# rebots-online/InstantIR

Measured on AMD Instinct MI355X. Metric: denoising steps/sec at 1024x1024 (InstantIR step: previewer UNet + LCM + Aggregator + UNet, CFG), higher is better.
Workload: dtype f16 (fp32 accumulate)

## Files before the change

### instantir_amd/csrc/gemm_conv.hip

```cpp
#include "common.h"
#include "gemm_geo.h"
#include "../../include/instantir_hip.h"
#include <stdlib.h>
#include <type_traits>

namespace {

using iir::Geo;

constexpr int BK = 64;
#ifndef IIR_NO_PIN
#define IIR_PIN() __builtin_amdgcn_sched_barrier(0)
#else
#define IIR_PIN() ((void)0)
#endif
constexpr int PF_TOUCHES = 4;
#define IIR_DEFAULT_STAGES 2
#ifndef IIR_T1_MIN
#define IIR_T1_MIN 384
#endif
#ifndef IIR_T2_MIN
#define IIR_T2_MIN 256
#endif


__device__ __forceinline__ void ln_merge(float& n, float& mean, float& m2, float nb, float mb, float m2b) {
    const float tot = n + nb, d = mb - mean;
    mean += d * (nb / tot);
    m2 += m2b + d * d * (n * nb / tot);
    n = tot;
}

constexpr int vmcnt_imm(int n) { return (n & 15) | 0x0F70 | ((n >> 4) << 14); }

template <int N>
__device__ __forceinline__ void wait_vm_lgkm_and_barrier() {
#ifdef IIR_DBG_NO_BARRIER
    asm volatile("s_waitcnt vmcnt(%0) lgkmcnt(0)" ::"n"(N) : "memory");
#else
    asm volatile("s_waitcnt vmcnt(%0) lgkmcnt(0)\n\ts_barrier" ::"n"(N) : "memory");
#endif
}

template <int N>
__device__ __forceinline__ void wait_vm_and_barrier() {
#ifdef IIR_DBG_NO_BARRIER
    asm volatile("s_waitcnt vmcnt(%0)" ::"n"(N) : "memory");
#else
    asm volatile("s_waitcnt vmcnt(%0)\n\ts_barrier" ::"n"(N) : "memory");
#endif
}

template <typename E, int BM, int BN, int ST, bool CONV, int WAVES_M = 2, bool W8 = false, bool LW = false, bool F8 = false>
__global__ __launch_bounds__(128 * WAVES_M * (LW ? 2 : 1), (WAVES_M == 2 ? 2 : 1)) void gemm_kernel(const Geo g) {
    static_assert(!(F8 && (W8 || CONV)), "the all-fp8 build covers the linear layers; W8 is the fp16-activation form");
    static_assert(!(W8 && CONV), "the fp8-weight build covers the linear layers only");
    static_assert(!(LW && W8), "loader waves: fp16 / bf16 operands only");
    using E4 = typename ET<E>::x4;
    using E8 = typename ET<E>::x8;
    constexpr int NW = WAVES_M * 2;
    constexpr int NT = 64 * NW * (LW ? 2 : 1);
    constexpr int WM = BM / WAVES_M, WN = BN / 2;
    constexpr int MI = WM / 16, NI = WN / 16;
    constexpr int B_GROUPS = W8 ? BN / 16 : BN / 8;
    constexpr int A_INST = BM / 8 / NW, B_INST = (B_GROUPS + NW - 1) / NW;
    constexpr int B_STAGE_BYTES = W8 ? BN * 64 : BN * 128;
    constexpr int RING_BYTES = ST * (BM * 128 + B_STAGE_BYTES);
    extern __shared__ __attribute__((aligned(16))) char smem[];
    f16* As = (f16*)smem;
    f16* Bs = As + ST * BM * BK;
    constexpr int LOADS = A_INST + B_INST;
    constexpr int SCRATCH_BYTES = 256 * NW * (LW ? 2 : 1);
    float2* rowstat = (float2*)(smem + RING_BYTES + SCRATCH_BYTES);
    constexpr int LNP_OFF = (BM * (2 * BN + 32) + 15) / 16 * 16;
    constexpr bool LN_OUT_FITS = LNP_OFF + BM * (BN / 8) * 8 <= RING_BYTES;
    constexpr int GN_RG = NT / (BN / 8);
    constexpr bool GN_OUT_FITS = BM % 64 == 0 && LNP_OFF + GN_RG * BN * 8 <= RING_BYTES && BN <= NT;

    const int tid = threadIdx.x;
    const int lane = tid & 63;
    const int wave_all = __builtin_amdgcn_readfirstlane(tid >> 6);
    const bool loader = LW && wave_all >= NW;
    const int wave = loader ? wave_all - NW : wave_all;
    const int wm = wave >> 1, wn = wave & 1;

    const int kz = (g.splitk == 2 && blockIdx.x >= (gridDim.x >> 1)) ? 1 : 0;
    int tm, tn;
    {
        const int bid = kz ? (int)blockIdx.x - (int)(gridDim.x >> 1) : (int)blockIdx.x, xcd = bid & 7, local = bid >> 3;
        const int rx = xcd % g.xm, ry = xcd / g.xm;
        tm = rx * g.rm + local % g.rm;
        tn = ry * g.rn + local / g.rm;
        if (tm >= g.tiles_m || tn >= g.tiles_n) return;
    }
    const int m0 = tm * BM, n0 = tn * BN;

    const int srow = lane >> 3;
    const int schunk = (lane & 7) ^ srow;
    const f16* a_src[A_INST];
    int a_pix_y[A_INST], a_pix_x[A_INST];
    const f16* a_img[A_INST];
#pragma unroll
    for (int i = 0; i < A_INST; ++i) {
        int m = m0 + (i * NW + wave) * 8 + srow;
        if (m >= g.M) m = g.M - 1;
        if (!CONV) {
            a_src[i] = g.A + (long)m * g.lda + schunk * 8;
        } else {
            const int hw = g.Ho * g.Wo;
            const int img = m / hw, rem = m - img * hw;
            const int oy = rem / g.Wo, ox = rem - oy * g.Wo;
            a_img[i] = g.A + (long)img * g.x_img_stride + schunk * 8;
            a_pix_y[i] = oy * g.stride - g.pad;
            a_pix_x[i] = ox * g.stride - g.pad;
        }
    }
    const f16* b_src[B_INST];
#pragma unroll
    for (int i = 0; i < B_INST; ++i) {
        if (!W8) {
            int n = n0 + (i * NW + wave) * 8 + srow;
            if (n >= g.N) n = g.N - 1;
            b_src[i] = g.W + (long)n * g.K + schunk * 8;
        } else {
            const int r = (i * NW + wave) * 16 + (lane >> 2);
            int n = n0 + r;
            if (n >= g.N) n = g.N - 1;
            b_src[i] = (const f16*)((const char*)g.W + (long)n * g.K + (((lane & 3) ^ ((r >> 2) & 3)) * 16));
        }
    }

    const f16* cv_ptr[CONV ? A_INST : 1];
    int cv_inc[CONV ? A_INST : 1];
    int cv_c0 = 0, cv_tap = 0;
    auto conv_tap = [&](int tap) {
        const int ky = tap / g.ks, kx = tap - ky * g.ks;
#pragma unroll
        for (int i = 0; i < (CONV ? A_INST : 0); ++i) {
            const int iy = a_pix_y[i] + ky, ix = a_pix_x[i] + kx;
            bool ok;
            long pix;
            if (g.ups) {
                ok = (iy >= 0) & (iy < 2 * g.H) & (ix >= 0) & (ix < 2 * g.Wd);
                pix = (long)(iy >> 1) * g.Wd + (ix >> 1);
            } else {
                ok = (iy >= 0) & (iy < g.H) & (ix >= 0) & (ix < g.Wd);
                pix = (long)iy * g.Wd + ix;
            }
            cv_ptr[i] = ok ? a_img[i] + pix * g.lda : g.zero + (lane & 7) * 8;
            cv_inc[i] = ok ? BK : 0;
        }
    };
    auto conv_seek = [&](int kt) {
        const int k0 = kt * BK;
        cv_tap = k0 / g.Cin;
        cv_c0 = k0 - cv_tap * g.Cin;
        conv_tap(cv_tap);
#pragma unroll
        for (int i = 0; i < (CONV ? A_INST : 0); ++i) cv_ptr[i] += cv_inc[i] ? cv_c0 : 0;
    };
// ... 466 lines not shown
    } else {
#pragma unroll
        for (int j = 0; j < NI; ++j) {
            const int n = n0 + wn * WN + j * 16 + fq * 4;
            const bool in_n = n < g.N;
            float sc[4] = {1.f, 1.f, 1.f, 1.f}, c0[4] = {0.f, 0.f, 0.f, 0.f}, c1[4] = {0.f, 0.f, 0.f, 0.f};
            if ((W8 || F8) && in_n) { const f32x4 ws = *(const f32x4*)(g.wscale + n); for (int t = 0; t < 4; ++t) sc[t] = ws[t] * g.a_scale; }
            for (int t = 0; t < 4; ++t) { c1[t] = pre_c1[j][t]; c0[t] = (float)pre_c0[j][t]; }
#pragma unroll
            for (int i = 0; i < MI; ++i) {
                const int lr = lrs[i];
                float a[4];
                for (int t = 0; t < 4; ++t) a[t] = (W8 || F8) ? acc[i][j][t] * sc[t] : acc[i][j][t];
                for (int t = 0; t < 4; ++t) a[t] = fmaf(a[t], rss[i].x, fmaf(rss[i].y, c1[t], c0[t]));
                float b[4];
                for (int t = 0; t < 4; ++t) b[t] = __shfl_xor(a[t], 32, 64);
                if (g.epi == IIR_EPI_GEGLU) {
                    if (!in_n) continue;
                    const bool gate = fq >= 2;
                    const int lco = (wn * WN + j * 16) / 2 + (fq & 1) * 4 + (gate ? 2 : 0);
                    const float v0 = gate ? b[2] : a[0], v1 = gate ? b[3] : a[1], g0 = gate ? a[2] : b[0], g1 = gate ? a[3] : b[1];
                    typedef E E2 __attribute__((ext_vector_type(2)));
                    E2 o2 = {(E)(v0 * gelu_erf_f(g0)), (E)(v1 * gelu_erf_f(g1))};
                    *(E2*)(ct + lr * cs + lco * 2) = o2;
                    continue;
                }
                if (fq >= 2 || !in_n) continue;
                const int lco = (wn * WN + j * 16) / 2 + fq * 4;
                long mr = ms[i];
                if (CONV && g.res_img_rows) { const int hw = g.Ho * g.Wo, img = ms[i] / hw; mr = (long)img * g.res_img_rows + (ms[i] - img * hw); }
                E4 o;
                {
                    E4 h = *(const E4*)(g.res + mr * g.ldr + n0 / 2 + lco);
                    for (int t = 0; t < 4; ++t) o[t] = (E)((float)h[t] * (a[t] + 1.0f) + b[t]);
                }
                *(E4*)(ct + lr * cs + lco * 2) = o;
            }
        }
    }
    }
    asm volatile("s_waitcnt lgkmcnt(0)\n\ts_barrier" ::: "memory");

    auto touch_next_weights = [&]() {
#ifdef IIR_DBG_NO_TOUCH
        return;
#endif
        const int per = (g.pf_lines + (int)gridDim.x - 1) / (int)gridDim.x;
        const long l0 = (long)blockIdx.x * per, last = g.pf_lines - 1;
        char* scratch = smem + RING_BYTES + wave_all * 256;
#pragma unroll
        for (int i = 0; i < PF_TOUCHES; ++i) {
            long l = l0 + min(tid + i * NT, per - 1);
            if (l > last) l = last;
            __builtin_amdgcn_global_load_lds((const GLOBAL_AS void*)(g.pf + l * 128), (LDS_AS void*)scratch, 4, 0, 0);
        }
    };
    auto write_out = [&](auto cpr_tag) {
        constexpr int CPR = decltype(cpr_tag)::value;
        constexpr int TOTAL = BM * CPR, CH = (TOTAL + NT - 1) / NT;
        const int no_tile = paired ? n0 / 2 : n0, No = paired ? g.N / 2 : g.N;
        const bool use_res = g.res && !paired;
        const bool remap = CONV && (g.y_img_rows | g.res_img_rows);
        const bool tr_tile = g.Ct && no_tile >= g.tr_from;
        const bool tr_mixed = g.Ct && !tr_tile && no_tile + CPR * 8 > g.tr_from;
        const bool inside = m0 + BM <= g.M && no_tile + CPR * 8 <= No && !remap;
        const bool fast = !tr_tile && !tr_mixed && g.c_vec && (!use_res || g.r_vec) && inside;
        if (tr_tile && inside && g.ct_vec && !use_res) {
            constexpr int RC = BM / 8, TOTAL_T = (CPR * 8) * RC, CH_T = (TOTAL_T + NT - 1) / NT;
            touch_next_weights();
#pragma unroll
            for (int k = 0; k < CH_T; ++k) {
                const int idx = tid + k * NT;
                if (TOTAL_T % NT != 0 && idx >= TOTAL_T) break;
                const int c = idx / RC, rc = idx - c * RC;
                E8 o;
#pragma unroll
                for (int t = 0; t < 8; ++t) o[t] = (E)((float)*(const E*)(ct + (rc * 8 + t) * cs + c * 2) * g.out_scale);
                *(E8*)(g.Ct + (long)(no_tile + c - g.tr_from) * g.ldct + m0 + rc * 8) = o;
            }
            return;
        }
        if constexpr (GN_OUT_FITS && CPR == BN / 8) {
        if (fast && g.gn_out && !paired) {
            constexpr int RG = NT / CPR, RPT = (64 + RG - 1) / RG;
            const int cc = tid % CPR, rg = tid / CPR;
            const bool active = rg < RG;
            float2* part = (float2*)(smem + LNP_OFF);
            touch_next_weights();
#pragma unroll 1
            for (int half = 0; half < BM / 64; ++half) {
                E8 rr[RPT];
                if (use_res) {
#pragma unroll
                    for (int j = 0; j < RPT; ++j) {
                        const int r = half * 64 + min(rg + j * RG, 63);
                        rr[j] = *(const E8*)(g.res + (long)(m0 + r) * g.ldr + no_tile + min(cc, CPR - 1) * 8);
                    }
                }
                float k0[8], s8[8], q8[8];
#pragma unroll
                for (int t = 0; t < 8; ++t) { k0[t] = 0.f; s8[t] = 0.f; q8[t] = 0.f; }
                int cnt = 0;
#pragma unroll
                for (int j = 0; j < RPT; ++j) {
                    const int rl = rg + j * RG;
                    if (active && rl < 64) {
                        const int r = half * 64 + rl;
                        const E8 v = *(const E8*)(ct + r * cs + cc * 16);
                        E8 o;
                        for (int t = 0; t < 8; ++t) o[t] = (E)(((float)v[t] + (use_res ? (float)rr[j][t] : 0.f)) * g.out_scale);
                        iir::store16(g.C, ((long)(m0 + r) * g.ldc + no_tile + cc * 8) * 2, o, g.st_wt != 0);
                        for (int t = 0; t < 8; ++t) {
                            const float f = (float)o[t];
                            if (j == 0) k0[t] = f;
                            const float d = f - k0[t];
                            s8[t] += d; q8[t] = fmaf(d, d, q8[t]);
                        }
                        ++cnt;
                    }
                }
                if (active) {
                    const float inv = 1.0f / (float)cnt;
#pragma unroll
                    for (int t = 0; t < 8; ++t)
                        part[rg * BN + cc * 8 + t] = make_float2(k0[t] + s8[t] * inv, fmaxf(q8[t] - s8[t] * s8[t] * inv, 0.f));
                }
                __syncthreads();
                if (tid < BN) {
                    float n = 0.f, mean = 0.f, m2 = 0.f;
#pragma unroll 4
                    for (int q = 0; q < RG; ++q) {
                        const float2 pq = part[q * BN + tid];
                        const float nb = (float)((64 - q + RG - 1) / RG);
                        const float tot = n + nb, d = pq.x - mean;
                        mean += d * (nb / tot);
                        m2 += pq.y + d * d * (n * nb / tot);
                        n = tot;
                    }
                    ((float2*)g.gn_out)[(long)(m0 / 64 + half) * g.N + n0 + tid] = make_float2(mean, m2);
                }
                __syncthreads();
            }
            return;
        }
        }
        if (fast) {
            E8 o[CH];
            if (use_res) {
                E8 rr[CH];
#pragma unroll
                for (int k = 0; k < CH; ++k) {
                    const int c = min(tid + k * NT, TOTAL - 1), r = c / CPR, cc = c - r * CPR;
                    rr[k] = *(const E8*)(g.res + (long)(m0 + r) * g.ldr + no_tile + cc * 8);
                }
#pragma unroll
                for (int k = 0; k < CH; ++k) {
                    const int c = min(tid + k * NT, TOTAL - 1), r = c / CPR, cc = c - r * CPR;
                    const E8 v = *(const E8*)(ct + r * cs + cc * 16);
                    for (int t = 0; t < 8; ++t) o[k][t] = (E)(((float)v[t] + (float)rr[k][t]) * g.out_scale);
                }
            } else {
#pragma unroll
                for (int k = 0; k < CH; ++k) {
                    const int c = min(tid + k * NT, TOTAL - 1), r = c / CPR, cc = c - r * CPR;
                    const E8 v = *(const E8*)(ct + r * cs + cc * 16);
                    for (int t = 0; t < 8; ++t) o[k][t] = (E)((float)v[t] * g.out_scale);
                }
            }
            touch_next_weights();
#pragma unroll
            for (int k = 0; k < CH; ++k) {
                const int c = tid + k * NT, r = c / CPR, cc = c - r * CPR;
                if (TOTAL % NT != 0 && c >= TOTAL) break;
                if constexpr (std::is_same<E, f16>::value) {
                    if (g.c_fp8) { *(long*)((char*)g.C + (long)(m0 + r) * g.ldc + no_tile + cc * 8) = iir_fp8x8(o[k]); continue; }
                }
                iir::store16(g.C, ((long)(m0 + r) * g.ldc + no_tile + cc * 8) * 2, o[k], g.st_wt != 0);
            }
            if constexpr (LN_OUT_FITS) {
                if (g.ln_out) {
                    float2* lnp = (float2*)(smem + LNP_OFF);
#pragma unroll
                    for (int k = 0; k < CH; ++k) {
                        const int c = tid + k * NT;
                        if (TOTAL % NT != 0 && c >= TOTAL) break;
                        float f[8], sum = 0.f, q = 0.f;
#pragma unroll
                        for (int t = 0; t < 8; ++t) { f[t] = (float)o[k][t]; sum += f[t]; }
                        const float mu = sum * 0.125f;
#pragma unroll
                        for (int t = 0; t < 8; ++t) { const float d = f[t] - mu; q = fmaf(d, d, q); }
                        lnp[c] = make_float2(mu, q);
                    }
                    __syncthreads();
                    if (tid < BM) {
                        float2 acc2 = lnp[tid * CPR];
                        float mean = acc2.x, m2 = acc2.y;
#pragma unroll
                        for (int j = 1; j < CPR; ++j) {
                            const float2 pj = lnp[tid * CPR + j];
                            const float d = pj.x - mean;
                            mean += d * (1.0f / (float)(j + 1));
                            m2 += pj.y + d * d * (8.0f * (float)j / (float)(j + 1));
                        }
                        ((float2*)g.ln_out)[(long)tn * g.M + m0 + tid] = make_float2(mean, m2);
                    }
                }
            }
        } else {
            touch_next_weights();
#pragma unroll 1
            for (int c = tid; c < TOTAL; c += NT) {
                const int r = c / CPR, cc = c - r * CPR;
                const int m = m0 + r, n = no_tile + cc * 8;
                if (m >= g.M || n >= No) continue;
                long mc = m, mr = m;
                if (remap) {
                    const int hw = g.Ho * g.Wo, img = m / hw, rem = m - img * hw;
                    if (g.y_img_rows) mc = (long)img * g.y_img_rows + rem;
                    if (g.res_img_rows) mr = (long)img * g.res_img_rows + rem;
                }
                const E* tp = (const E*)(ct + r * cs + cc * 16);
#pragma unroll 1
                for (int t = 0; t < 8 && n + t < No; ++t) {
                    float v = (float)tp[t];
                    if (g.Ct && n + t >= g.tr_from) { ((E*)g.Ct)[(long)(n + t - g.tr_from) * g.ldct + mc] = (E)(v * g.out_scale); continue; }
                    if (use_res) v += (float)((const E*)g.res)[mr * g.ldr + n + t];
                    ((E*)g.C)[mc * g.ldc + n + t] = (E)(v * g.out_scale);
                }
            }
        }
    };
    if (paired) write_out(std::integral_constant<int, BN / 16>{});
    else write_out(std::integral_constant<int, BN / 8>{});
    asm volatile("s_waitcnt vmcnt(0)" ::: "memory");
}

template <typename E, int BM, int BN, int ST, int WAVES_M = 2, bool W8 = false, bool LW = false, bool F8 = false>
int launch_t(const Geo& g0, bool conv, hipStream_t stream) {
    Geo g = g0;
    g.tiles_m = (g.M + BM - 1) / BM;
    g.tiles_n = (g.N + BN - 1) / BN;
    static const size_t dbg_pad = getenv("IIR_DBG_LDS_PAD") ? (size_t)atoi(getenv("IIR_DBG_LDS_PAD")) : 0;
    const size_t lds = ST * (BM * 128 + (W8 ? BN * 64 : BN * 128)) + 256 * WAVES_M * 2 * (LW ? 2 : 1) + BM * 8 + dbg_pad;
    if (g.c_fp8) {
        if (conv || g.M % BM || g.N % BN || g.ldc % 8 || (uintptr_t)g.C % 8 || g.Ct || g.c_f32 || g.ln_out || g.gn_out || g.res_img_rows || g.y_img_rows ||
            (g.res && !g.r_vec) || g.dtype != IIR_DT_F16) return IIR_EINVAL;
        g.c_vec = 1; g.st_wt = 0;
    }
    if (g.gn_out) {
        constexpr int RINGB = ST * (BM * 128 + (W8 ? BN * 64 : BN * 128)), NTH = 128 * WAVES_M * (LW ? 2 : 1);
        constexpr bool fits = BM % 64 == 0 && BN <= NTH && (BM * (2 * BN + 32) + 15) / 16 * 16 + (NTH / (BN / 8)) * BN * 8 <= RINGB;
        if (!fits || g.epi != IIR_EPI_PLAIN || g.c_f32 || g.Ct || g.splitk == 2 || g.ln_out || g.M % BM || g.N % BN || !g.c_vec || (g.res && !g.r_vec) ||
            (conv && (g.y_img_rows | g.res_img_rows)))
            return IIR_EINVAL;
    }
    if (g.ln_out) {
        constexpr bool fits = (BM * (2 * BN + 32) + 15) / 16 * 16 + BM * (BN / 8) * 8 <= ST * (BM * 128 + (W8 ? BN * 64 : BN * 128));
        if (!fits || conv || g.epi != IIR_EPI_PLAIN || g.c_f32 || g.Ct || g.splitk == 2 || g.M % BM || g.N % BN || !g.c_vec || (g.res && !g.r_vec))
            return IIR_EINVAL;
    }
    double best = -1.;
    static const int force_xm = getenv("IIR_XM") ? atoi(getenv("IIR_XM")) : 0;
    const double row_bytes = (double)g.K * 2.;
    for (int xm = 1; xm <= 8; xm *= 2) {
        if (force_xm && xm != force_xm) continue;
        const int xn = 8 / xm;
        const int rm = (g.tiles_m + xm - 1) / xm, rn = (g.tiles_n + xn - 1) / xn;
        const double a_bytes = (double)rm * BM * row_bytes, w_bytes = (double)rn * BN * row_bytes;
        const int cols_per_group = rm >= 64 ? 1 : 64 / rm;
        const double groups = (double)((rn + cols_per_group - 1) / cols_per_group);
        double cost = (a_bytes <= 3.0 * 1048576. ? a_bytes : a_bytes * groups) + w_bytes;
        cost += ((double)rm * rn * 8 - (double)g.tiles_m * g.tiles_n) * 8. * BK * (BM + BN);
        if (best < 0. || cost < best) { best = cost; g.xm = xm; g.rm = rm; g.rn = rn; }
    }
    const dim3 grid(8 * g.rm * g.rn * (g.splitk == 2 ? 2 : 1)), block(128 * WAVES_M * (LW ? 2 : 1));
    auto ensure_lds = [&](const void* fn) -> bool {
        static unsigned long long done[64] = {};
        int dev = 0;
        if (hipGetDevice(&dev) != hipSuccess || dev < 0 || dev >= 64) return false;
        const int slot = conv ? 1 : 0;
        if (done[dev] & (1ull << slot)) return true;
        if (hipFuncSetAttribute(fn, hipFuncAttributeMaxDynamicSharedMemorySize, (int)lds) != hipSuccess) return false;
        done[dev] |= 1ull << slot;
        return true;
    };
    if constexpr (F8) {
        if (conv || g.splitk == 2) return IIR_EINVAL;
        if (!ensure_lds((const void*)gemm_kernel<E, BM, BN, ST, false, WAVES_M, false, LW, true>)) return IIR_ELAUNCH;
        iir_launch(gemm_kernel<E, BM, BN, ST, false, WAVES_M, false, LW, true>, grid, block, lds, stream, g);
        return iir_launch_status();
    } else if constexpr (W8) {
        if (!ensure_lds((const void*)gemm_kernel<E, BM, BN, ST, false, WAVES_M, true>)) return IIR_ELAUNCH;
        iir_launch(gemm_kernel<E, BM, BN, ST, false, WAVES_M, true>, grid, block, lds, stream, g);
        return iir_launch_status();
    } else if constexpr (LW) {
        if (g.splitk == 2) return IIR_EINVAL;
        if (conv) {
            if (!ensure_lds((const void*)gemm_kernel<E, BM, BN, ST, true, WAVES_M, false, true>)) return IIR_ELAUNCH;
            iir_launch(gemm_kernel<E, BM, BN, ST, true, WAVES_M, false, true>, grid, block, lds, stream, g);
        } else {
            if (!ensure_lds((const void*)gemm_kernel<E, BM, BN, ST, false, WAVES_M, false, true>)) return IIR_ELAUNCH;
            iir_launch(gemm_kernel<E, BM, BN, ST, false, WAVES_M, false, true>, grid, block, lds, stream, g);
        }
        return iir_launch_status();
    } else
    if (conv) {
        if (!ensure_lds((const void*)gemm_kernel<E, BM, BN, ST, true, WAVES_M>)) return IIR_ELAUNCH;
        iir_launch(gemm_kernel<E, BM, BN, ST, true, WAVES_M>, grid, block, lds, stream, g);
    } else {
        if (!ensure_lds((const void*)gemm_kernel<E, BM, BN, ST, false, WAVES_M>)) return IIR_ELAUNCH;
        iir_launch(gemm_kernel<E, BM, BN, ST, false, WAVES_M>, grid, block, lds, stream, g);
    }
    return iir_launch_status();
}

template <int BM, int BN, int ST, int WAVES_M = 2>
int launch(const Geo& g, bool conv, hipStream_t stream) {
    if (g.f8) {
        if constexpr (WAVES_M == 2 && (ST == 2 || (ST == 3 && BM == 64 && BN == 160))) {
            if (conv || g.dtype != IIR_DT_F16) return IIR_EINVAL;
            return launch_t<f16, BM, BN, ST, WAVES_M, false, false, true>(g, false, stream);
        } else return IIR_EINVAL;
    }
    if (g.wscale) {
        if constexpr (WAVES_M == 2 && (ST == 2 || (ST == 3 && BM == 64 && BN == 160))) {
            if (conv || g.dtype != IIR_DT_F16 || g.splitk == 2) return IIR_EINVAL;
            return launch_t<f16, BM, BN, ST, WAVES_M, true>(g, false, stream);
        } else return IIR_EINVAL;
    }
    if (g.dtype == IIR_DT_BF16) {
        if constexpr (ST == 2 && WAVES_M == 2) return launch_t<bf16, BM, BN, ST, WAVES_M>(g, conv, stream);
        else return IIR_EINVAL;
    }
    return launch_t<f16, BM, BN, ST, WAVES_M>(g, conv, stream);
}

template <int BM, int BN, int ST>
int lw_launch(const Geo& g, bool conv, hipStream_t stream) {
    if (g.f8) {
        if constexpr (ST == 3 && BM == 64 && BN == 160) { if (conv) return IIR_EINVAL; return launch_t<f16, BM, BN, ST, 2, false, true, true>(g, false, stream); }
        else return IIR_EINVAL;
    }
    if (g.wscale || g.dtype != IIR_DT_F16 || g.splitk == 2) return IIR_EINVAL;
    if constexpr (ST == 3) return launch_t<f16, BM, BN, ST, 2, false, true>(g, conv, stream);
    else { if (conv) return IIR_EINVAL; return launch_t<f16, BM, BN, ST, 2, false, true>(g, false, stream); }
}

struct TileShape { int bm, bn; };
constexpr TileShape kTiles[] = {{0, 0}, {128, 128}, {128, 64}, {64, 64}, {128, 160}, {64, 160}, {256, 128}, {128, 320}, {256, 256}, {32, 160}};

int one_per_cu_min_k() { static const int v = [] { const char* e = getenv("IIR_T5_MINK"); return e ? atoi(e) : 1280; }(); return v; }
int one_per_cu_stages() { static const int v = [] { const char* e = getenv("IIR_T5_STAGES"); return e ? atoi(e) : 3; }(); return v; }

int pick_tile(int M, int N, bool paired, int K = 0) {
    if (K >= one_per_cu_min_k() && (long)((M + 63) / 64) * ((N + 159) / 160) <= 256) return 5;
    long best = -1;
    int pick = 1;
    for (int t = 1; t <= 5; ++t) {
        const long blocks = (long)((M + kTiles[t].bm - 1) / kTiles[t].bm) * ((N + kTiles[t].bn - 1) / kTiles[t].bn);
        const long cost = ((blocks + 511) / 512) * 2 * (kTiles[t].bm + kTiles[t].bn);
        if (best < 0 || cost < best || (cost == best && kTiles[t].bm * kTiles[t].bn > kTiles[pick].bm * kTiles[pick].bn)) {
            best = cost;
            pick = t;
        }
    }
    return pick;
}

constexpr long SK_CNT_BYTES = 4096;
long splitk_ws_bytes(int M, int N) {
    const long t = (long)((M + 127) / 128) * ((N + 159) / 160);
    return t * 2 <= 256 ? SK_CNT_BYTES + t * 2 * 128 * 160 * (long)sizeof(float) : 0;
}

bool uses_splitk(int M, int N, int K, long ws_bytes) {
    const long need = splitk_ws_bytes(M, N);
    return K >= one_per_cu_min_k() && (K / BK) % 2 == 0 && need > 0 && ws_bytes >= need;
}

bool gemm8_auto(const Geo& g, bool conv) {
    static const bool g8_on = !(getenv("IIR_G8") && atoi(getenv("IIR_G8")) == 0);
    return g8_on && !conv && (g.f8 ? 2 * g.K : g.K) >= 640 && (long)(g.M / 256) * (g.N / 320) >= 256 && iir::gemm8_covers(g, 320);
}

int dispatch(const Geo& g, bool conv, int tile, hipStream_t stream) {
    if (g.xa_on) return conv ? IIR_EINVAL : launch<64, 128, 3>(g, false, stream);
    if (tile == 0 && g.sk_slabs && !g.ln_out && !g.ln_in && !g.gn_out && g.dtype == IIR_DT_F16 && uses_splitk(g.M, g.N, g.K, g.sk_bytes)) {
        Geo g2 = g;
        g2.splitk = 2;
        return launch<128, 160, 3>(g2, conv, stream);
    }
    if (tile == 0 && gemm8_auto(g, conv)) return iir::gemm8_launch(g, 320, stream);
    if (tile == 91 || tile == 92) return conv ? IIR_EINVAL : iir::gemm8_launch(g, tile == 91 ? 320 : 256, stream);
    if (tile == 0) tile = pick_tile(g.M, g.N, g.epi != IIR_EPI_PLAIN, g.f8 ? 2 * g.K : g.K);
    if (tile < 10) {
        const long blocks = (long)((g.M + kTiles[tile].bm - 1) / kTiles[tile].bm) * ((g.N + kTiles[tile].bn - 1) / kTiles[tile].bn);
        const bool one_per_cu = tile == 5 && blocks <= 256 && (g.f8 ? 2 * g.K : g.K) >= one_per_cu_min_k() && g.dtype == IIR_DT_F16;
        const int stages = one_per_cu ? one_per_cu_stages() : IIR_DEFAULT_STAGES;
        static const bool lw_on = !(getenv("IIR_T5_LW") && atoi(getenv("IIR_T5_LW")) == 0);
        static const bool lw_conv = !(getenv("IIR_T5_LWCONV") && atoi(getenv("IIR_T5_LWCONV")) == 0);
        static const bool lw2 = getenv("IIR_T5_LW2") && atoi(getenv("IIR_T5_LW2")) == 1;
        if (one_per_cu && lw2 && !conv && !g.wscale && g.splitk != 2) tile = 75;
        else
        if (one_per_cu && lw_on && (!conv || (lw_conv && stages == 3)) && (!g.wscale || (g.f8 && stages == 3)) && g.splitk != 2 && stages >= 3 && stages <= 5) tile = stages == 3 ? 55 : stages == 4 ? 65 : 85;
        else
        tile += 10 * stages;
    }
    switch (tile) {
        case 21: return launch<128, 128, 2>(g, conv, stream);
        case 31: return launch<128, 128, 3>(g, conv, stream);
        case 22: return launch<128, 64, 2>(g, conv, stream);
        case 32: return launch<128, 64, 3>(g, conv, stream);
        case 23: return launch<64, 64, 2>(g, conv, stream);
        case 33: return launch<64, 64, 3>(g, conv, stream);
        case 24: return launch<128, 160, 2>(g, conv, stream);
        case 25: return launch<64, 160, 2>(g, conv, stream);
        case 35: return launch<64, 160, 3>(g, conv, stream);
        case 45: return launch<64, 160, 4>(g, conv, stream);
        case 55: return lw_launch<64, 160, 3>(g, conv, stream);
        case 65: return lw_launch<64, 160, 4>(g, conv, stream);
        case 75: return lw_launch<64, 160, 2>(g, conv, stream);
        case 85: return lw_launch<64, 160, 5>(g, conv, stream);
        case 34: return launch<128, 160, 3>(g, conv, stream);
        case 56: return launch<64, 160, 3, 4>(g, conv, stream);
        case 66: return launch<64, 160, 4, 4>(g, conv, stream);
        case 57: return launch<128, 160, 3, 4>(g, conv, stream);
        case 47: return launch<128, 160, 2, 4>(g, conv, stream);
        case 42: return launch<128, 64, 4>(g, conv, stream);
        case 26: return launch<256, 128, 2, 4>(g, conv, stream);
        case 36: return launch<256, 128, 3, 4>(g, conv, stream);
        case 29: return launch<32, 160, 2>(g, conv, stream);
        case 27: return launch<128, 320, 2, 4>(g, conv, stream);
        case 90:
            if (g.epi == IIR_EPI_PLAIN) return IIR_EINVAL;
            return launch<256, 320, 2, 4>(g, conv, stream);
        case 28:
            if (g.epi == IIR_EPI_PLAIN && !g.c_f32) return IIR_EINVAL;
            return launch<256, 256, 2, 4>(g, conv, stream);
        default: return IIR_EINVAL;
    }
}

void finish_geo(Geo& g) {
    static const int wt = getenv("IIR_ST_WT") ? atoi(getenv("IIR_ST_WT")) : 1;
    g.st_wt = wt && ((long)g.M * g.ldc * 2 < (1L << 31));
    if (g.pf_lines <= 0) { g.pf = (const char*)g.W; g.pf_lines = 1; }
    g.c_vec = (g.ldc % 8 == 0) && ((uintptr_t)g.C % 16 == 0);
    g.r_vec = g.res && (g.ldr % 8 == 0) && ((uintptr_t)g.res % 16 == 0);
}

}

extern "C" int iir_gemm_tile_bn(int32_t tile) { tile %= 10; return (tile >= 1 && tile <= 9) ? kTiles[tile].bn : -1; }

extern "C" int64_t iir_gemm_splitk_workspace_bytes(int32_t M, int32_t N) { return splitk_ws_bytes(M, N); }
extern "C" int iir_gemm_uses_splitk(int32_t M, int32_t N, int32_t K, int64_t ws_bytes) { return uses_splitk(M, N, K, ws_bytes) ? 1 : 0; }

extern "C" int iir_gemm_pick_tile(int32_t M, int32_t N, int32_t K, int32_t paired) { return pick_tile(M, N, paired != 0, K); }

extern "C" int iir_gemm_ln_parts(int32_t M, int32_t N, int32_t K) {
    const int t = pick_tile(M, N, false, K);
    const int bm = kTiles[t].bm, bn = kTiles[t].bn;
    if (t < 1 || t > 5 || M % bm || N % bn || N / bn > 8) return 0;
    return N / bn;
}

static int fill_gemm_geo(const iir_gemm_desc* d, Geo& g);

extern "C" int iir_gemm_gn_supported(int32_t M, int32_t N, int32_t K, int32_t is_conv) {
    if (M <= 0 || N <= 0 || K <= 0 || M % 64) return 0;
    const int t = pick_tile(M, N, false, K);
    if (t < 1 || t > 5) return 0;
    const int bm = kTiles[t].bm, bn = kTiles[t].bn;
    if (M % bm || N % bn) return 0;
    const long blocks = (long)(M / bm) * (N / bn);
    const bool lw = t == 5 && blocks <= 256 && K >= one_per_cu_min_k() && one_per_cu_stages() == 3;
    const int st = lw ? 3 : IIR_DEFAULT_STAGES, nt = lw ? 512 : 256;
    const long ring = (long)st * (bm + bn) * 128, need = ((long)bm * (2 * bn + 32) + 15) / 16 * 16 + (long)(nt / (bn / 8)) * bn * 8;
    (void)is_conv;
    return bn <= nt && need <= ring ? 1 : 0;
}

extern "C" int iir_gemm_fp8_out_supported(int32_t M, int32_t N, int32_t K, int32_t paired) {
    if (M <= 0 || N <= 0 || K <= 0 || K % 128) return 0;
    const int t = pick_tile(M, N, paired != 0, K);
    if (t < 1 || t > 5) return 0;
    return (M % kTiles[t].bm == 0 && N % kTiles[t].bn == 0) ? 1 : 0;
}

extern "C" int iir_gemm_f16(const iir_gemm_desc* d, void* stream) {
    (void)hipGetLastError();
    Geo g{};
    const int rc = fill_gemm_geo(d, g);
    if (rc != IIR_OK) return rc;
    return dispatch(g, false, d->tile, (hipStream_t)stream);
}

extern "C" int iir_gemm_resolve_tile(const iir_gemm_desc* d) {
    Geo g{};
    if (fill_gemm_geo(d, g) != IIR_OK) return -1;
    if (g.xa_on) return 93;
    if (d->tile != 0) return d->tile;
    if (gemm8_auto(g, false)) return 91;
    return pick_tile(g.M, g.N, g.epi != IIR_EPI_PLAIN, g.f8 ? 2 * g.K : g.K);
}

static int fill_gemm_geo(const iir_gemm_desc* d, Geo& g) {
    if (!d || !d->A || !d->W || !d->C) return IIR_EINVAL;
    if (d->M <= 0 || d->N <= 0 || d->K <= 0 || d->K % BK) return IIR_EINVAL;
    if (d->N % 4 || d->lda % 8 || d->ldc % 4) return IIR_EINVAL;
    if (d->epi != IIR_EPI_PLAIN && (d->N % 16)) return IIR_EINVAL;
    if (d->epi == IIR_EPI_SFT && !d->res) return IIR_EINVAL;
    if (d->rowbias && d->rows_per_rb <= 0) return IIR_EINVAL;
    if (d->epi < IIR_EPI_PLAIN || d->epi > IIR_EPI_XATTN) return IIR_EINVAL;
    if (d->epi == IIR_EPI_XATTN) {
        const iir_attn_kv* kv = d->xattn_kv;
        if (!kv || d->dtype != IIR_DT_F16 || d->N % 128 || d->M % 64 || d->xattn_tq <= 0 || d->xattn_tq % 64 || d->M % d->xattn_tq) return IIR_EINVAL;
        if (d->res || d->rowbias || d->act || d->Ct || d->c_f32 || d->wscale || d->ln_stats_out || d->gn_stats_out || d->splitk_ws) return IIR_EINVAL;
        if (d->ldc % 8 || (uintptr_t)d->C % 16 || (d->tile != 0 && d->tile != 93)) return IIR_EINVAL;
        if (kv[0].Tkv < 1 || kv[0].Tkv > 80 || kv[1].Tkv < 1 || kv[1].Tkv > 64) return IIR_EINVAL;
        for (int sgm = 0; sgm < 2; ++sgm) {
            if (!kv[sgm].K || !kv[sgm].Vt || (uintptr_t)kv[sgm].K % 16 || (uintptr_t)kv[sgm].Vt % 16) return IIR_EINVAL;
            if (kv[sgm].ldk % 8 || kv[sgm].k_batch_stride % 8 || kv[sgm].ldvt % 8 || kv[sgm].vt_batch_stride % 8) return IIR_EINVAL;
            g.xa_k[sgm] = (const f16*)kv[sgm].K; g.xa_ldk[sgm] = kv[sgm].ldk; g.xa_kb[sgm] = kv[sgm].k_batch_stride;
            g.xa_vt[sgm] = (const f16*)kv[sgm].Vt; g.xa_ldvt[sgm] = kv[sgm].ldvt; g.xa_vb[sgm] = kv[sgm].vt_batch_stride;
            g.xa_tk[sgm] = kv[sgm].Tkv;
        }
        g.xa_on = 1; g.xa_tq = d->xattn_tq;
    }
    g.A = (const f16*)d->A; g.lda = d->lda; g.W = (const f16*)d->W; g.C = (f16*)d->C; g.ldc = d->ldc;
    g.M = d->M; g.N = d->N; g.K = d->K;
    g.bias = (const f16*)d->bias; g.rowbias = (const f16*)d->rowbias; g.ldrb = d->ldrb; g.rows_per_rb = d->rows_per_rb;
    g.res = (const f16*)d->res; g.ldr = d->ldr; g.epi = d->epi == IIR_EPI_XATTN ? IIR_EPI_PLAIN : d->epi; g.act = d->act;
    g.out_scale = d->out_scale == 0.f ? 1.f : d->out_scale;
    g.pf = (const char*)d->prefetch; g.pf_lines = d->prefetch ? (int)(d->prefetch_bytes / 128) : 0;
    finish_geo(g);
    if (d->dtype != IIR_DT_F16 && d->dtype != IIR_DT_BF16) return IIR_EINVAL;
    g.dtype = d->dtype;
    if (d->c_f32) {
        if (d->epi != IIR_EPI_PLAIN || d->bias || d->rowbias || d->res || d->Ct || d->act || d->ldc % 4 || (uintptr_t)d->C % 16 || d->splitk_ws) return IIR_EINVAL;
        g.c_f32 = 1;
    }
    if (d->wscale) {
        if (d->c_f32 || d->K % 64 || (uintptr_t)d->W % 16 || (uintptr_t)d->wscale % 16 || d->dtype != IIR_DT_F16) return IIR_EINVAL;
        g.wscale = (const float*)d->wscale;
        g.sk_slabs = nullptr;
    }
    if (d->c_fp8) {
        if (d->epi == IIR_EPI_XATTN || d->epi == IIR_EPI_SFT || d->c_f32 || d->Ct || d->ln_stats_out || d->gn_stats_out || d->dtype != IIR_DT_F16) return IIR_EINVAL;
        g.c_fp8 = 1;
    }
    g.a_scale = 1.f;
    if (d->a_fp8) {
        if (!d->wscale || d->K % 128 || d->lda % 16 || (uintptr_t)d->A % 16 || d->ln_stats_in || d->epi == IIR_EPI_XATTN || d->splitk_ws) return IIR_EINVAL;
        g.f8 = 1;
        g.a_scale = d->a_scale == 0.f ? 1.f : d->a_scale;
        g.K = d->K / 2; g.lda = d->lda / 2;
    }
    if (d->Ct) {
        if (d->epi != IIR_EPI_PLAIN || d->tr_from < 0 || d->tr_from >= d->N || d->tr_from % 8 || d->ldct < d->M) return IIR_EINVAL;
        g.Ct = (f16*)d->Ct; g.ldct = d->ldct; g.tr_from = d->tr_from;
        g.ct_vec = (d->ldct % 8 == 0) && ((uintptr_t)d->Ct % 16 == 0);
    }
    if (d->splitk_ws && d->splitk_ws_bytes > SK_CNT_BYTES) {
        g.sk_cnt = (int*)d->splitk_ws; g.sk_slabs = (float*)((char*)d->splitk_ws + SK_CNT_BYTES); g.sk_bytes = d->splitk_ws_bytes;
    }
    if (d->ln_stats_out) {
        if ((uintptr_t)d->ln_stats_out % 8 || d->c_f32 || d->Ct || d->epi != IIR_EPI_PLAIN) return IIR_EINVAL;
        g.ln_out = (float*)d->ln_stats_out;
    }
    if (d->gn_stats_out) {
        if ((uintptr_t)d->gn_stats_out % 8 || d->M % 64 || d->epi != IIR_EPI_PLAIN || d->c_f32 || d->Ct || d->ln_stats_out || d->wscale) return IIR_EINVAL;
        g.gn_out = (float*)d->gn_stats_out;
    }
    if (d->ln_stats_in) {
        if (!d->ln_colsum || d->ln_parts <= 0 || d->ln_parts > 8 || d->ln_part_cols <= 0 || (long)d->ln_parts * d->ln_part_cols != d->K || d->c_f32 ||
            (uintptr_t)d->ln_stats_in % 8 || (uintptr_t)d->ln_colsum % 16 || !(d->ln_eps > 0.f)) return IIR_EINVAL;
        g.ln_in = (const float*)d->ln_stats_in; g.ln_colsum = (const float*)d->ln_colsum;
        g.ln_parts = d->ln_parts; g.ln_part_cols = d->ln_part_cols; g.ln_eps = d->ln_eps;
    }
    return IIR_OK;
}

extern "C" int iir_conv2d_nhwc_f16(const iir_conv_desc* c, void* stream) {
    (void)hipGetLastError();
    if (!c || !c->X || !c->Wt || !c->Y || !c->zero_page) return IIR_EINVAL;
    if (c->ksize != 3 && c->ksize != 1) return IIR_EINVAL;
// ... 35 lines not shown
```

### instantir_amd/engine.py

```python
from __future__ import annotations

import os

from typing import Dict, List, Optional

import torch

from . import ops
from .config import UNetConfig
from .packing import conv_weight_nhwc, pair_rows
from .weights import skip_channels

F16 = torch.float16
CPAD = 64


class _NullOps:

    def __getattr__(self, name):
        return lambda *a, **k: None


class Arena:

# ... 198 lines not shown
        self.w["temb_all.w"] = torch.cat(ws, 0).contiguous()
        self.w["temb_all.b"] = torch.cat(bs, 0).contiguous()
        if self._ada:
            off, ws, bs = 0, [], []
            for key, w, b in self._ada:
                self._ada_slices[key] = slice(off, off + w.shape[0])
                off += w.shape[0]
                ws.append(w); bs.append(b)
            self.w["ada_all.w"] = torch.cat(ws, 0).contiguous()
            self.w["ada_all.b"] = torch.cat(bs, 0).contiguous()
        del self._temb, self._ada

    def _size_arena(self, fn):
        self.arena.buf, self.arena.off, self.arena.high = None, 0, 0
        self.arena_gen = getattr(self, "arena_gen", 0) + 1
        self.o = _NullOps()
        plain = self.w
        first = not self.units
        self._gnws = ops.gn_workspace(self.device, 64, self.cfg.norm_groups)
        if self._skws is None and os.environ.get("IIR_SPLITK", "0") == "1":
            self._skws = torch.zeros(4096 + 256 * 128 * 160 * 4, dtype=torch.uint8, device=self.device)
        if first:
            self._use_log = []
            self.w = _RecDict(plain, lambda k: self._use_log.append(k))
        try:
            fn()
        finally:
            self.o = ops
            self.w = plain
        if first:
            self._consolidate_weights()
        self.arena.reserve(self.arena.high + 1024)
        self.arena.reset()

    def _consolidate_weights(self):
        order, seen, marks = [], set(), []
        for k in self._use_log:
            if isinstance(k, tuple):
                marks.append(len(order))
            elif k not in seen:
                seen.add(k)
                order.append(k)
        order += [k for k in self.w if k not in seen]
        order = [k for k in order if torch.is_tensor(self.w[k]) and self.w[k].dtype == F16]
        al = lambda n: (n + 127) // 128 * 128
        offs, tot = [], 0
        for k in order:
            offs.append(tot)
            tot += al(self.w[k].numel())
        arena = torch.empty(tot, dtype=F16, device=self.device)
        for k, off in zip(order, offs):
            t = self.w[k]
            v = arena[off:off + t.numel()].view(t.shape)
            v.copy_(t)
            self.w[k] = v
        self._warena = arena
        self.units = [None]
        self._use_log = None

    def _unit(self, name):
        if self._use_log is not None:
            self._use_log.append(("unit", name))

    import os as _os
    PF_MULT = float(_os.environ.get("IIR_PF_MULT", "1"))
    PF_LOOKAHEAD = int(_os.environ.get("IIR_PF_MB", "0")) << 20

    def _pf(self, wt):
        if not self.inkernel_prefetch or self._warena is None or self.o is not ops:
            return None
        base, end = self._warena.data_ptr(), self._warena.data_ptr() + self._warena.numel() * 2
        n = wt.numel() * 2
        lo = wt.data_ptr() + n + self.PF_LOOKAHEAD
        if lo < base or lo >= end or n < (256 << 10):
            return None
        return (lo, min(int(n * self.PF_MULT), end - lo))

    def _begin(self):
        self.arena.reset()

    def _gn_alloc(self, rows, hw, C, K, conv):
        if not self.gn_fuse or hw % 64 or self.arena.dtype != F16 or not ops.gn_supported(rows, C, K, conv):
            return None
        if (hw // 64) * (C // 32) > ops.GN_PARTIALS_MAX:
            return None
        return self.arena.alloc(rows // 64 * C, 4).view(torch.float32).view(rows // 64, C, 2)

    @staticmethod
    def _gn_of(x):
        return getattr(x, "_gn_parts", None)

    def _resnet(self, path, x, R, H, W, temb_all, out=None, eps=1e-5):
        self._unit(path)
        o, w, A = self.o, self.w, self.arena
        HW = H * W
        cin = x.shape[1]
        cout = w[path + ".conv1.w"].shape[0]
        if out is None:
            out = A.alloc(R * HW, cout)
        p_out = self._gn_alloc(R * HW, HW, cout, 9 * cout, True) if self._skws is None else None
        m = A.mark()
        h = A.alloc(R * HW, cin)
        o.groupnorm(x, h, R, HW, w[path + ".norm1.g"], w[path + ".norm1.b"], eps, True, self.cfg.norm_groups, self._gnws,
                    partials=self._gn_of(x))
        h2 = A.alloc(R * HW, cout)
        p2 = self._gn_alloc(R * HW, HW, cout, 9 * cin, True) if self._skws is None else None
        o.conv2d(h.view(R, H, W, cin), w[path + ".conv1.w"], h2, bias=w[path + ".conv1.b"],
                 rowbias=temb_all[:, self._temb_slices[path]], rows_per_rb=HW, prefetch=self._pf(w[path + ".conv1.w"]),
                 splitk_ws=self._skws, gn_out=p2)
        h3 = A.alloc(R * HW, cout)
        o.groupnorm(h2, h3, R, HW, w[path + ".norm2.g"], w[path + ".norm2.b"], eps, True, self.cfg.norm_groups, self._gnws, partials=p2)
        if (path + ".conv_shortcut.w") in w:
            sc = A.alloc(R * HW, cout)
            o.gemm(x, w[path + ".conv_shortcut.w"], sc, bias=w[path + ".conv_shortcut.b"])
        else:
            sc = x
        o.conv2d(h3.view(R, H, W, cout), w[path + ".conv2.w"], out, bias=w[path + ".conv2.b"], res=sc,
                 prefetch=self._pf(w[path + ".conv2.w"]), splitk_ws=self._skws, gn_out=p_out)
        if p_out is not None:
            out._gn_parts = p_out
        A.release(m)
        return out

    def _tblock(self, p, h, R, T, heads, st, ada, lnst=None, last=False):
        self._unit(p)
        o, w, A = self.o, self.w, self.arena
        C = h.shape[1]
        M = R * T
        m = A.mark()
        fold = lnst is not None
        if self.fp8_act and not fold and C % 128 == 0 and isinstance(w[p + ".attn1.qkv.w"], ops.Fp8Weight) and h.dtype == F16:
            self._tblock_fp8(p, h, R, T, heads, st)
            A.release(m)
            return
        n = None if fold else A.alloc(M, C)
        qk = A.alloc(M, 2 * C)
        vt = A.alloc(C, M)
        if fold:
            wqkv = w[p + ".attn1.qkv.lnw"]
            o.gemm(h, wqkv, qk, bias=w[p + ".attn1.qkv.lnb"], prefetch=self._pf(wqkv), out_t=(vt, 2 * C),
                   ln_in=(lnst, w[p + ".attn1.qkv.lncs"], 1e-5))
        else:
            o.layernorm(h, n, w[p + ".norm1.g"], w[p + ".norm1.b"], 1e-5)
            wqkv = w[p + ".attn1.qkv.w"]
            if self.fuse_qkv:
                o.gemm(n, wqkv, qk, prefetch=self._pf(wqkv), out_t=(vt, 2 * C))
            else:
                o.gemm(n, wqkv[:2 * C], qk, prefetch=self._pf(wqkv))
                o.gemm(wqkv[2 * C:], n, vt)
        a = A.alloc(M, C)
        o.attention(qk[:, :C], a, [(qk[:, C:], T, vt, T, T)], R, heads, T, q_prescaled=True)
        o.gemm(a, w[p + ".attn1.to_out.0.w"], h, bias=w[p + ".attn1.to_out.0.b"], res=h,
               prefetch=self._pf(w[p + ".attn1.to_out.0.w"]), ln_out=lnst)
        if self.cross:
            q = qk[:, :C]
            cfg = self.cfg
            nip, ipad = cfg.num_ip_tokens, (cfg.num_ip_tokens + 7) // 8 * 8
            kv = st["kv"][p]
            ipk, ipvt = kv["ipk"], kv["ipvt"]
            segs = [(kv["tk"], cfg.text_len, kv["tvt"], kv["tpad"], cfg.text_len), (ipk, nip, ipvt, ipad, nip)]
            wq = w[p + (".attn2.to_q.lnw" if fold else ".attn2.to_q.w")]
            fuse = (self.xattn_fuse and cfg.head_dim == 64 and C % 128 == 0 and T % 64 == 0 and cfg.text_len <= 80 and nip <= 64 and h.dtype == F16
                    and not isinstance(wq, ops.Fp8Weight))
            if not fold:
                o.layernorm(h, n, w[p + ".norm2.g"], w[p + ".norm2.b"], 1e-5)
            src = h if fold else n
            kw = dict(bias=w[p + ".attn2.to_q.lnb"], ln_in=(lnst, w[p + ".attn2.to_q.lncs"], 1e-5)) if fold else {}
# ... 418 lines not shown
```

Before: 16.98.

## Add 128x160 loader-wave tile for mid-size GEMMs and centralize tile resolution

Adds a new tile variant (id 54, BM=128, BN=160, three stages, loader waves) that is chosen automatically for f16 GEMMs whose 64-row tiling would exceed one block per CU while 128-row tiling fits. The GN-stats epilogue is split across two thread slices, each handling alternate 64-row halves, so the larger tile can still emit groupnorm partials. Tile selection logic is factored into a shared resolve_tile used by dispatch and the support queries, so ln/gn/fp8 capability checks agree with the actual kernel chosen. The engine's GN partial limit now uses the configured group count instead of a hardcoded 32. Larger tiles reduce block count and improve weight reuse but may lower occupancy or change split behavior.

```diff
diff --git a/instantir_amd/csrc/gemm_conv.hip b/instantir_amd/csrc/gemm_conv.hip
--- a/instantir_amd/csrc/gemm_conv.hip
+++ b/instantir_amd/csrc/gemm_conv.hip
@@ -32,6 +32,13 @@
 }
 
 constexpr int vmcnt_imm(int n) { return (n & 15) | 0x0F70 | ((n >> 4) << 14); }
+
+constexpr int gn_par(int bm, bool lw) { return lw && bm == 128 ? 2 : 1; }
+constexpr bool gn_out_fits(int bm, int bn, int st, int nt, bool lw, bool w8 = false) {
+    const int gnt = nt / gn_par(bm, lw);
+    const long ring = (long)st * (bm * 128 + (w8 ? bn * 64 : bn * 128));
+    return bm % 64 == 0 && bn <= gnt && ((long)bm * (2 * bn + 32) + 15) / 16 * 16 + (long)gn_par(bm, lw) * (gnt / (bn / 8)) * bn * 8 <= ring;
+}
 
 template <int N>
 __device__ __forceinline__ void wait_vm_lgkm_and_barrier() {
@@ -74,8 +81,9 @@
     float2* rowstat = (float2*)(smem + RING_BYTES + SCRATCH_BYTES);
     constexpr int LNP_OFF = (BM * (2 * BN + 32) + 15) / 16 * 16;
     constexpr bool LN_OUT_FITS = LNP_OFF + BM * (BN / 8) * 8 <= RING_BYTES;
-    constexpr int GN_RG = NT / (BN / 8);
-    constexpr bool GN_OUT_FITS = BM % 64 == 0 && LNP_OFF + GN_RG * BN * 8 <= RING_BYTES && BN <= NT;
+    constexpr int GN_PAR = gn_par(BM, LW), GN_NT = NT / GN_PAR;
+    constexpr int GN_RG = GN_NT / (BN / 8);
+    constexpr bool GN_OUT_FITS = gn_out_fits(BM, BN, ST, NT, LW, W8);
 
     const int tid = threadIdx.x;
     const int lane = tid & 63;
@@ -708,13 +716,14 @@
         }
         if constexpr (GN_OUT_FITS && CPR == BN / 8) {
         if (fast && g.gn_out && !paired) {
-            constexpr int RG = NT / CPR, RPT = (64 + RG - 1) / RG;
-            const int cc = tid % CPR, rg = tid / CPR;
+            constexpr int RG = GN_RG, RPT = (64 + RG - 1) / RG;
+            const int sl = GN_PAR == 1 ? 0 : tid / GN_NT, lt = tid - sl * GN_NT;
+            const int cc = lt % CPR, rg = lt / CPR;
             const bool active = rg < RG;
-            float2* part = (float2*)(smem + LNP_OFF);
+            float2* part = (float2*)(smem + LNP_OFF) + sl * RG * BN;
             touch_next_weights();
 #pragma unroll 1
-            for (int half = 0; half < BM / 64; ++half) {
+            for (int half = sl; half < BM / 64; half += GN_PAR) {
                 E8 rr[RPT];
                 if (use_res) {
 #pragma unroll
@@ -752,18 +761,18 @@
                         part[rg * BN + cc * 8 + t] = make_float2(k0[t] + s8[t] * inv, fmaxf(q8[t] - s8[t] * s8[t] * inv, 0.f));
                 }
                 __syncthreads();
-                if (tid < BN) {
+                if (lt < BN) {
                     float n = 0.f, mean = 0.f, m2 = 0.f;
 #pragma unroll 4
                     for (int q = 0; q < RG; ++q) {
-                        const float2 pq = part[q * BN + tid];
+                        const float2 pq = part[q * BN + lt];
                         const float nb = (float)((64 - q + RG - 1) / RG);
                         const float tot = n + nb, d = pq.x - mean;
                         mean += d * (nb / tot);
                         m2 += pq.y + d * d * (n * nb / tot);
                         n = tot;
                     }
-                    ((float2*)g.gn_out)[(long)(m0 / 64 + half) * g.N + n0 + tid] = make_float2(mean, m2);
+                    ((float2*)g.gn_out)[(long)(m0 / 64 + half) * g.N + n0 + lt] = make_float2(mean, m2);
                 }
                 __syncthreads();
             }
@@ -875,8 +884,7 @@
         g.c_vec = 1; g.st_wt = 0;
     }
     if (g.gn_out) {
-        constexpr int RINGB = ST * (BM * 128 + (W8 ? BN * 64 : BN * 128)), NTH = 128 * WAVES_M * (LW ? 2 : 1);
-        constexpr bool fits = BM % 64 == 0 && BN <= NTH && (BM * (2 * BN + 32) + 15) / 16 * 16 + (NTH / (BN / 8)) * BN * 8 <= RINGB;
+        constexpr bool fits = gn_out_fits(BM, BN, ST, 128 * WAVES_M * (LW ? 2 : 1), LW, W8);
         if (!fits || g.epi != IIR_EPI_PLAIN || g.c_f32 || g.Ct || g.splitk == 2 || g.ln_out || g.M % BM || g.N % BN || !g.c_vec || (g.res && !g.r_vec) ||
             (conv && (g.y_img_rows | g.res_img_rows)))
             return IIR_EINVAL;
@@ -994,6 +1002,30 @@
     return pick;
 }
 
+struct Resolved { int id, bm, bn, st, nt; bool lw; };
+
+Resolved resolve_tile(int M, int N, int K, bool conv, int dtype, bool wscale, bool f8, int tile) {
+    const bool f16 = dtype == IIR_DT_F16;
+    if (tile == 0) {
+        static const bool t4_lw = !(getenv("IIR_T4_LW") && atoi(getenv("IIR_T4_LW")) == 0);
+        if (t4_lw && f16 && !wscale && !f8 && K >= one_per_cu_min_k() && M % 128 == 0 && N % 160 == 0 &&
+            (long)(M / 128) * (N / 160) <= 256 && (long)(M / 64) * (N / 160) > 256 && pick_tile(M, N, false, K) == 5)
+            return {54, 128, 160, 3, 512, true};
+        tile = pick_tile(M, N, false, K);
+    }
+    const int bm = kTiles[tile].bm, bn = kTiles[tile].bn;
+    const long blocks = (long)((M + bm - 1) / bm) * ((N + bn - 1) / bn);
+    const bool one_per_cu = tile == 5 && blocks <= 256 && K >= one_per_cu_min_k() && f16;
+    const int stages = one_per_cu ? one_per_cu_stages() : IIR_DEFAULT_STAGES;
+    static const bool lw_on = !(getenv("IIR_T5_LW") && atoi(getenv("IIR_T5_LW")) == 0);
+    static const bool lw_conv = !(getenv("IIR_T5_LWCONV") && atoi(getenv("IIR_T5_LWCONV")) == 0);
+    static const bool lw2 = getenv("IIR_T5_LW2") && atoi(getenv("IIR_T5_LW2")) == 1;
+    if (one_per_cu && lw2 && !conv && !wscale) return {75, bm, bn, 2, 512, true};
+    if (one_per_cu && lw_on && (!conv || (lw_conv && stages == 3)) && (!wscale || (f8 && stages == 3)) && stages >= 3 && stages <= 5)
+        return {stages == 3 ? 55 : stages == 4 ? 65 : 85, bm, bn, stages, 512, true};
+    return {tile + 10 * stages, bm, bn, stages, tile >= 6 && tile <= 8 ? 512 : 256, false};
+}
+
 constexpr long SK_CNT_BYTES = 4096;
 long splitk_ws_bytes(int M, int N) {
     const long t = (long)((M + 127) / 128) * ((N + 159) / 160);
@@ -1019,20 +1051,7 @@
     }
     if (tile == 0 && gemm8_auto(g, conv)) return iir::gemm8_launch(g, 320, stream);
     if (tile == 91 || tile == 92) return conv ? IIR_EINVAL : iir::gemm8_launch(g, tile == 91 ? 320 : 256, stream);
-    if (tile == 0) tile = pick_tile(g.M, g.N, g.epi != IIR_EPI_PLAIN, g.f8 ? 2 * g.K : g.K);
-    if (tile < 10) {
-        const long blocks = (long)((g.M + kTiles[tile].bm - 1) / kTiles[tile].bm) * ((g.N + kTiles[tile].bn - 1) / kTiles[tile].bn);
-        const bool one_per_cu = tile == 5 && blocks <= 256 && (g.f8 ? 2 * g.K : g.K) >= one_per_cu_min_k() && g.dtype == IIR_DT_F16;
-        const int stages = one_per_cu ? one_per_cu_stages() : IIR_DEFAULT_STAGES;
-        static const bool lw_on = !(getenv("IIR_T5_LW") && atoi(getenv("IIR_T5_LW")) == 0);
-        static const bool lw_conv = !(getenv("IIR_T5_LWCONV") && atoi(getenv("IIR_T5_LWCONV")) == 0);
-        static const bool lw2 = getenv("IIR_T5_LW2") && atoi(getenv("IIR_T5_LW2")) == 1;
-        if (one_per_cu && lw2 && !conv && !g.wscale && g.splitk != 2) tile = 75;
-        else
-        if (one_per_cu && lw_on && (!conv || (lw_conv && stages == 3)) && (!g.wscale || (g.f8 && stages == 3)) && g.splitk != 2 && stages >= 3 && stages <= 5) tile = stages == 3 ? 55 : stages == 4 ? 65 : 85;
-        else
-        tile += 10 * stages;
-    }
+    if (tile < 10) tile = resolve_tile(g.M, g.N, g.f8 ? 2 * g.K : g.K, conv, g.dtype, g.wscale != nullptr, g.f8 != 0, tile).id;
     switch (tile) {
         case 21: return launch<128, 128, 2>(g, conv, stream);
         case 31: return launch<128, 128, 3>(g, conv, stream);
@@ -1044,6 +1063,7 @@
         case 25: return launch<64, 160, 2>(g, conv, stream);
         case 35: return launch<64, 160, 3>(g, conv, stream);
         case 45: return launch<64, 160, 4>(g, conv, stream);
+        case 54: return lw_launch<128, 160, 3>(g, conv, stream);
         case 55: return lw_launch<64, 160, 3>(g, conv, stream);
         case 65: return lw_launch<64, 160, 4>(g, conv, stream);
         case 75: return lw_launch<64, 160, 2>(g, conv, stream);
@@ -1086,33 +1106,26 @@
 extern "C" int iir_gemm_pick_tile(int32_t M, int32_t N, int32_t K, int32_t paired) { return pick_tile(M, N, paired != 0, K); }
 
 extern "C" int iir_gemm_ln_parts(int32_t M, int32_t N, int32_t K) {
-    const int t = pick_tile(M, N, false, K);
-    const int bm = kTiles[t].bm, bn = kTiles[t].bn;
-    if (t < 1 || t > 5 || M % bm || N % bn || N / bn > 8) return 0;
-    return N / bn;
+    if (M <= 0 || N <= 0 || K <= 0) return 0;
+    const Resolved r = resolve_tile(M, N, K, false, IIR_DT_F16, false, false, 0);
+    if (M % r.bm || N % r.bn || N / r.bn > 8) return 0;
+    return N / r.bn;
 }
 
 static int fill_gemm_geo(const iir_gemm_desc* d, Geo& g);
 
 extern "C" int iir_gemm_gn_supported(int32_t M, int32_t N, int32_t K, int32_t is_conv) {
     if (M <= 0 || N <= 0 || K <= 0 || M % 64) return 0;
-    const int t = pick_tile(M, N, false, K);
-    if (t < 1 || t > 5) return 0;
-    const int bm = kTiles[t].bm, bn = kTiles[t].bn;
-    if (M % bm || N % bn) return 0;
-    const long blocks = (long)(M / bm) * (N / bn);
-    const bool lw = t == 5 && blocks <= 256 && K >= one_per_cu_min_k() && one_per_cu_stages() == 3;
-    const int st = lw ? 3 : IIR_DEFAULT_STAGES, nt = lw ? 512 : 256;
-    const long ring = (long)st * (bm + bn) * 128, need = ((long)bm * (2 * bn + 32) + 15) / 16 * 16 + (long)(nt / (bn / 8)) * bn * 8;
-    (void)is_conv;
-    return bn <= nt && need <= ring ? 1 : 0;
+    const Resolved r = resolve_tile(M, N, K, is_conv != 0, IIR_DT_F16, false, false, 0);
+    if (M % r.bm || N % r.bn) return 0;
+    return gn_out_fits(r.bm, r.bn, r.st, r.nt, r.lw) ? 1 : 0;
 }
 
 extern "C" int iir_gemm_fp8_out_supported(int32_t M, int32_t N, int32_t K, int32_t paired) {
     if (M <= 0 || N <= 0 || K <= 0 || K % 128) return 0;
-    const int t = pick_tile(M, N, paired != 0, K);
-    if (t < 1 || t > 5) return 0;
-    return (M % kTiles[t].bm == 0 && N % kTiles[t].bn == 0) ? 1 : 0;
+    (void)paired;
+    const Resolved r = resolve_tile(M, N, K, false, IIR_DT_F16, true, true, 0);
+    return (M % r.bm == 0 && N % r.bn == 0) ? 1 : 0;
 }
 
 extern "C" int iir_gemm_f16(const iir_gemm_desc* d, void* stream) {
@@ -1129,7 +1142,7 @@
     if (g.xa_on) return 93;
     if (d->tile != 0) return d->tile;
     if (gemm8_auto(g, false)) return 91;
-    return pick_tile(g.M, g.N, g.epi != IIR_EPI_PLAIN, g.f8 ? 2 * g.K : g.K);
+    return resolve_tile(g.M, g.N, g.f8 ? 2 * g.K : g.K, false, g.dtype, g.wscale != nullptr, g.f8 != 0, 0).id;
 }
 
 static int fill_gemm_geo(const iir_gemm_desc* d, Geo& g) {
diff --git a/instantir_amd/engine.py b/instantir_amd/engine.py
--- a/instantir_amd/engine.py
+++ b/instantir_amd/engine.py
@@ -304,7 +304,7 @@
     def _gn_alloc(self, rows, hw, C, K, conv):
         if not self.gn_fuse or hw % 64 or self.arena.dtype != F16 or not ops.gn_supported(rows, C, K, conv):
             return None
-        if (hw // 64) * (C // 32) > ops.GN_PARTIALS_MAX:
+        if (hw // 64) * (C // self.cfg.norm_groups) > ops.GN_PARTIALS_MAX:
             return None
         return self.arena.alloc(rows // 64 * C, 4).view(torch.float32).view(rows // 64, C, 2)
 
```

New measurement: 17.36, median of 6. 2.3% higher.
